# hassony2/handobjectconsist

Hardware: AMD Instinct MI355X
Metric: trainmeshwarp iters/sec (render+warp, B=64, 256x256) (higher is better)
Workload: dtype f32; 1 GPU; trainmeshwarp.py consist step, per-GPU B=64, 256x256, hand 778v/1552f + object 1002v/2000f (7104 faces after fill-back), ResNet-18 fp32 (MIOpen convolutions, channels-last, + fused HIP BatchNorm/ReLU/residual/max-pool kernels), Adam; global_batch=64, image_size=256, parallelism=dp1

## Files before the change

### handobjectconsist_amd/_lib.py

```python
import ctypes
import os

import torch

_HERE = os.path.dirname(os.path.abspath(__file__))
LIB_PATH = os.environ.get("HOC_LIB_PATH") or os.path.join(_HERE, "libmeshraster_hip.so")
ABI_VERSION = 9
FLAG_REFERENCE_ALGO = 1
FLAG_SPARSE_TILES = 2
FLAG_OUTPUT_ZEROED = 4
FLAG_TILE_PER_WORKGROUP = 8
FLAG_TILE_LIST_CLEARED = 16
FLAG_FORCE_PARTS = 1 << 24
FLAG_ONE_WORKGROUP_PER_IMAGE = 32 << 24
FLAG_PARTS_IN_ONE_LAUNCH = 64 << 24
FLAG_PLAIN_DIVISIONS = 4096 << 8
FLAG_FORCE_GATHER = 32 << 8
FLAG_COUNT_PIXEL_MAP_TERMS = 1024 << 8
CRITERION_L1 = 0
CRITERION_L2 = 1
DTYPE_F32, DTYPE_BF16, DTYPE_U8 = 0, 1, 2
DTYPE_CODES = {torch.float32: DTYPE_F32, torch.bfloat16: DTYPE_BF16, torch.uint8: DTYPE_U8}
IMAGE_DTYPES = (torch.float32, torch.bfloat16)
MASK_DTYPES = (torch.float32, torch.uint8)
# ... 71 lines not shown
    "mr_flow_pair_forward_tiles_typed": (_I, [_P] * 4 + [_L] + [_P] * 12 + [_I, _P, _L, _P, _P, _P, _I, _I, _I, _I, _F, _F, _F, _P, _P, _L, _L, _P, _I, _I, _I]),
    "mr_flow_pair_forward_grad_tiles_typed": (_I, [_P] * 4 + [_L] + [_P] * 12 + [_I, _P, _L, _P, _P, _P, _I, _I, _I, _I, _F, _F, _F, _P, _P, _L, _L, _P, _P, _P, _P, _P, _I, _I, _I]),
    "mr_pair_step_struct_bytes": (_L, []),
    "mr_pair_step_field_offsets": (_I, [_P, _I]),
    "mr_pair_step_sizes": (_I, [_P, _P, _P, _P]),
    "mr_pair_step_forward": (_I, [_P, _P]),
    "mr_pair_step_backward": (_I, [_P, _P]),
    "mr_frames_to_batch_workspace_bytes": (_L, [_I, _I, _I]),
    "mr_frames_to_batch": (_I, [_P] * 3 + [_F] * 6 + [_P, _L, _P, _P] + [_I] * 6 + [_P]),
    "mr_frames_to_batch_typed": (_I, [_P] * 3 + [_F] * 6 + [_P, _L, _P, _P] + [_I] * 6 + [_P, _I, _I]),
    "mr_frames_color_augment_workspace_bytes": (_L, [_I, _I, _I]),
    "mr_frames_color_augment": (_I, [_P] * 7 + [_L, _I, _I, _I, _P]),
    "mr_jpeg_info": (_I, [_P, _L, _P]),
    "mr_jpeg_packed_bytes": (_L, [_I] * 5),
    "mr_jpeg_entropy_decode": (_I, [_P, _L, _P, _L]),
    "mr_jpeg_reconstruct_workspace_bytes": (_L, [_I] * 6),
    "mr_jpeg_reconstruct": (_I, [_P] + [_I] * 6 + [_P, _P, _L, _P]),
    "mr_png_packed_bytes": (_L, [_I] * 3),
    "mr_png_unfilter_workspace_bytes": (_L, [_I] * 4),
    "mr_png_unfilter": (_I, [_P] + [_I] * 4 + [_P, _P, _P]),
    "mr_bn_act_forward": (_I, [_P] * 6 + [_F, _I, _I, _I, _P, _I, _I, _I, _P]),
    "mr_bn_act_backward_workspace_bytes": (_L, [_I, _I]),
    "mr_bn_act_backward": (_I, [_P] * 8 + [_F, _I, _I, _I] + [_P] * 5 + [_L, _I, _I, _I, _P]),
    "mr_stem_pool_forward": (_I, [_P] * 5 + [_F, _I, _I, _P, _P, _I, _I, _I, _I, _P]),
    "mr_stem_pool_backward_workspace_bytes": (_L, [_I, _I, _I, _I]),
    "mr_stem_pool_backward": (_I, [_P] * 8 + [_F, _I, _I] + [_P] * 4 + [_L, _I, _I, _I, _I, _P]),
}

_lib = None


def load():
    global _lib
    if _lib is not None:
        return _lib
    if not os.path.exists(LIB_PATH):
        raise RuntimeError(
            f"{LIB_PATH} is missing: the HIP extension has not been built. Run "
            "`python -c 'import __graft_entry__ as g; g.build()'` (or `python handobjectconsist_amd/build.py`). "
            "There is no CPU / PyTorch fallback for the render + warp path."
        )
    lib = ctypes.CDLL(LIB_PATH)
    for name, (res, args) in SIGNATURES.items():
        try:
            fn = getattr(lib, name)
        except AttributeError as e:
            raise RuntimeError(f"{LIB_PATH} does not export {name}; rebuild it") from e
# ... 86 lines not shown
```

### handobjectconsist_amd/csrc/frozen_bn.hip

```cpp
#include "mr_common.hpp"

namespace mr {

__device__ __forceinline__ float relu_nan(float z) { return z > 0.0f ? z : (z != z ? z : 0.0f); }


struct BnParams {
    const void* x;
    const void* residual;
    const float* weight;
    const float* bias;
    const float* mean;
    const float* var;
    float eps;
    int relu;
    int N, C, HW, split;
    void* y;
    const void* grad_y;
    const void* grad_y2;
    void* grad_x;
    void* grad_residual;
    float* partial;
};

// ... 184 lines not shown
#pragma unroll
        for (int i = 0; i < 4; i++) { red[threadIdx.x][i] = sg[i]; red[threadIdx.x][4 + i] = sgx[i]; }
        __syncthreads();
        if (threadIdx.x < groups) {
            float t[8] = {0, 0, 0, 0, 0, 0, 0, 0};
            for (int r = 0; r < rows; r++)
#pragma unroll
                for (int i = 0; i < 8; i++) t[i] += red[r * groups + threadIdx.x][i];
#pragma unroll
            for (int i = 0; i < 4; i++) {
                p.partial[(int64_t)(c0 + i) * gridDim.x + blockIdx.x] = t[i];
                p.partial[(int64_t)(p.C + c0 + i) * gridDim.x + blockIdx.x] = t[4 + i];
            }
        }
    }
}

static inline bool bn_nhwc_ok(int C) { return C >= 4 && C <= 1024 && (1024 % C) == 0; }

static inline int bn_nhwc_blocks(int64_t pixels, int C) {
    const int rows = 256 / (C / 4);
    const int64_t need = (pixels + rows - 1) / rows;
    return (int)(need < BN_NHWC_BLOCKS ? (need < 1 ? 1 : need) : BN_NHWC_BLOCKS);
}

static inline int bn_split(int N, int C) {
    int s = (4096 + C - 1) / C;
    if (s < 1) s = 1;
    if (s > N) s = N;
    return s;
}

static inline bool bn_aligned(const void* p, int bytes) { return (reinterpret_cast<uintptr_t>(p) & (uintptr_t)(bytes - 1)) == 0; }

template <bool BACKWARD>
static void bn_launch(const BnParams& p, int act_dtype, bool vec, hipStream_t s) {
    const dim3 grid((unsigned)(p.C * p.split));
    if (act_dtype == 0) {
        if (vec) hipLaunchKernelGGL((bn_act_kernel<float, true, BACKWARD>), grid, dim3(256), 0, s, p);
        else hipLaunchKernelGGL((bn_act_kernel<float, false, BACKWARD>), grid, dim3(256), 0, s, p);
    } else {
        if (vec) hipLaunchKernelGGL((bn_act_kernel<bf16_t, true, BACKWARD>), grid, dim3(256), 0, s, p);
        else hipLaunchKernelGGL((bn_act_kernel<bf16_t, false, BACKWARD>), grid, dim3(256), 0, s, p);
    }
}

// ... 67 lines not shown
    if (channels_last) {
        if (!bn_aligned(x, vb) || !bn_aligned(grad_y, vb) || !bn_aligned(grad_y2, vb) || !bn_aligned(grad_x, vb) ||
            !bn_aligned(residual, vb) ||
            !bn_aligned(grad_residual, vb))
            return MR_ERR_BADARG;
        slots = bn_nhwc_blocks((int64_t)batch_size * plane, channels);
        const dim3 grid((unsigned)slots);
        if (act_dtype == 0) hipLaunchKernelGGL((bn_act_nhwc_kernel<float, true>), grid, dim3(256), 0, (hipStream_t)stream, p);
        else hipLaunchKernelGGL((bn_act_nhwc_kernel<bf16_t, true>), grid, dim3(256), 0, (hipStream_t)stream, p);
    } else {
        const bool vec = plane % 4 == 0 && bn_aligned(x, vb) && bn_aligned(grad_y, vb) && bn_aligned(grad_y2, vb) &&
                         bn_aligned(grad_x, vb) &&
                         bn_aligned(residual, vb) && bn_aligned(grad_residual, vb);
        bn_launch<true>(p, act_dtype, vec, (hipStream_t)stream);
    }
    MR_CHECK_LAUNCH();
    if (want_params) {
        hipLaunchKernelGGL(bn_finish_kernel, dim3((unsigned)channels), dim3(256), 0, (hipStream_t)stream, p.partial,
                           running_var, eps, grad_weight, grad_bias, channels, slots);
        MR_CHECK_LAUNCH();
    }
    return MR_OK;
}
```

### handobjectconsist_amd/csrc/stem_pool.hip

```cpp
#include "mr_common.hpp"

namespace mr {

__device__ __forceinline__ float sp_relu_nan(float z) { return z > 0.0f ? z : (z != z ? z : 0.0f); }


struct StemParams {
    const void* x;
    const float* weight;
    const float* bias;
    const float* mean;
    const float* var;
    float eps;
    int N, C, H, W, OH, OW;
    int tiles_x, tiles_y;
    void* y;
    const void* grad_y;
    const void* grad_y2;
    void* grad_x;
    float* partial;
    unsigned char* argmax;
};

constexpr int SP_TX = 32, SP_TY = 16;
// ... 305 lines not shown
            sg[i] += gm;
            sgx[i] += gm * d;
        }
        sp_store4<T>(static_cast<T*>(p.grad_x), ip * p.C + c0, out);
    }
    if (p.partial) {
#pragma unroll
        for (int i = 0; i < 4; i++) { red[threadIdx.x][i] = sg[i]; red[threadIdx.x][4 + i] = sgx[i]; }
        __syncthreads();
        if (threadIdx.x < groups) {
            float t[8] = {0, 0, 0, 0, 0, 0, 0, 0};
            for (int r = 0; r < rows; r++)
#pragma unroll
                for (int i = 0; i < 8; i++) t[i] += red[r * groups + threadIdx.x][i];
#pragma unroll
            for (int i = 0; i < 4; i++) {
                p.partial[(int64_t)(c0 + i) * gridDim.x + blockIdx.x] = t[i];
                p.partial[(int64_t)(p.C + c0 + i) * gridDim.x + blockIdx.x] = t[4 + i];
            }
        }
    }
}

static inline bool sp_nhwc_ok(int C) { return C >= 4 && C <= 1024 && (1024 % C) == 0; }
static inline int sp_nhwc_blocks(int64_t pixels, int C) {
    const int rows = 256 / (C / 4);
    const int64_t need = (pixels + rows - 1) / rows;
    return (int)(need < SP_NHWC_BLOCKS ? (need < 1 ? 1 : need) : SP_NHWC_BLOCKS);
}

static int stem_fill(StemParams& p, const void* x, const float* weight, const float* bias, const float* mean,
                     const float* var, float eps, int N, int C, int H, int W) {
    if (N < 0 || C < 0 || H < 0 || W < 0) return MR_ERR_BADARG;
    p.x = x; p.weight = weight; p.bias = bias; p.mean = mean; p.var = var; p.eps = eps;
    p.N = N; p.C = C; p.H = H; p.W = W;
    p.OH = H > 0 ? (H - 1) / 2 + 1 : 0;
    p.OW = W > 0 ? (W - 1) / 2 + 1 : 0;
    p.tiles_x = (p.OW + SP_TX - 1) / SP_TX;
    p.tiles_y = (p.OH + SP_TY - 1) / SP_TY;
    if ((int64_t)N * C * p.tiles_x * p.tiles_y > 0x7fffffff) return MR_ERR_BADARG;
    return MR_OK;
}

}

extern "C" int mr_stem_pool_forward(const void* x, const float* weight, const float* bias, const float* running_mean,
                                    const float* running_var, float eps, int act_dtype, int channels_last, void* y,
                                    unsigned char* argmax, int batch_size, int channels, int height, int width,
                                    mr_stream_t stream) {
    using namespace mr;
    if (act_dtype != 0 && act_dtype != 1) return MR_ERR_BADARG;
    if (channels_last && channels > 0 && !sp_nhwc_ok(channels)) return MR_ERR_BADARG;
    StemParams p{};
    const int rc = stem_fill(p, x, weight, bias, running_mean, running_var, eps, batch_size, channels, height, width);
    if (rc != MR_OK) return rc;
    if (batch_size == 0 || channels == 0 || height == 0 || width == 0) return MR_OK;
    if (!x || !weight || !bias || !running_mean || !running_var || !y) return MR_ERR_BADARG;
    p.y = y;
    if (channels_last) {
        const uintptr_t am = (uintptr_t)(act_dtype == 0 ? 15 : 7);
        if (!argmax || (reinterpret_cast<uintptr_t>(x) & am) || (reinterpret_cast<uintptr_t>(y) & am) ||
            (reinterpret_cast<uintptr_t>(argmax) & 3))
            return MR_ERR_BADARG;
        p.argmax = argmax;
        const dim3 g((unsigned)sp_nhwc_blocks((int64_t)batch_size * p.OH * p.OW, channels));
        if (act_dtype == 0) hipLaunchKernelGGL(stem_pool_nhwc_forward_kernel<float>, g, dim3(256), 0, (hipStream_t)stream, p);
        else hipLaunchKernelGGL(stem_pool_nhwc_forward_kernel<bf16_t>, g, dim3(256), 0, (hipStream_t)stream, p);
        MR_CHECK_LAUNCH();
        return MR_OK;
    }
    const dim3 grid((unsigned)((int64_t)batch_size * channels * p.tiles_x * p.tiles_y));
    if (act_dtype == 0) hipLaunchKernelGGL(stem_pool_forward_kernel<float>, grid, dim3(256), 0, (hipStream_t)stream, p);
    else hipLaunchKernelGGL(stem_pool_forward_kernel<bf16_t>, grid, dim3(256), 0, (hipStream_t)stream, p);
    MR_CHECK_LAUNCH();
    return MR_OK;
}

extern "C" int64_t mr_stem_pool_backward_workspace_bytes(int batch_size, int channels, int height, int width) {
    using namespace mr;
    StemParams p{};
    if (stem_fill(p, nullptr, nullptr, nullptr, nullptr, nullptr, 0.0f, batch_size, channels, height, width) != MR_OK) return -1;
    const int64_t nchw = (int64_t)batch_size * p.tiles_x * p.tiles_y;
    return (int64_t)2 * channels * (nchw > SP_NHWC_BLOCKS ? nchw : SP_NHWC_BLOCKS) * 4 + 16;
}

extern "C" int mr_stem_pool_backward(const void* grad_y, const void* grad_y2, const void* x, const unsigned char* argmax,
                                     const float* weight, const float* bias, const float* running_mean, const float* running_var, float eps,
                                     int act_dtype, int channels_last, void* grad_x, float* grad_weight,
                                     float* grad_bias, void* workspace, int64_t workspace_bytes, int batch_size,
                                     int channels, int height, int width, mr_stream_t stream) {
    using namespace mr;
    if (act_dtype != 0 && act_dtype != 1) return MR_ERR_BADARG;
    if (channels_last && channels > 0 && !sp_nhwc_ok(channels)) return MR_ERR_BADARG;
    StemParams p{};
    const int rc = stem_fill(p, x, weight, bias, running_mean, running_var, eps, batch_size, channels, height, width);
    if (rc != MR_OK) return rc;
    if (channels == 0) return MR_OK;
    const bool want_params = grad_weight || grad_bias;
    if (batch_size == 0 || height == 0 || width == 0) {
        hipError_t e = hipSuccess;
        if (grad_weight) e = hipMemsetAsync(grad_weight, 0, (size_t)channels * 4, (hipStream_t)stream);
        if (e == hipSuccess && grad_bias) e = hipMemsetAsync(grad_bias, 0, (size_t)channels * 4, (hipStream_t)stream);
        return e == hipSuccess ? MR_OK : (int)e;
    }
    if (!grad_y || !x || !weight || !bias || !running_mean || !running_var || !grad_x) return MR_ERR_BADARG;
    if (want_params &&
        (!workspace || workspace_bytes < mr_stem_pool_backward_workspace_bytes(batch_size, channels, height, width)))
        return MR_ERR_BADARG;
    p.grad_y = grad_y; p.grad_y2 = grad_y2; p.grad_x = grad_x;
    p.partial = want_params ? static_cast<float*>(workspace) : nullptr;
    const int tiles = p.tiles_x * p.tiles_y;
    int64_t slots = (int64_t)batch_size * tiles;
    if (channels_last) {
        const uintptr_t am = (uintptr_t)(act_dtype == 0 ? 15 : 7);
        if (!argmax || (reinterpret_cast<uintptr_t>(x) & am) || (reinterpret_cast<uintptr_t>(grad_y) & am) ||
            (reinterpret_cast<uintptr_t>(grad_y2) & am) ||
            (reinterpret_cast<uintptr_t>(grad_x) & am) || (reinterpret_cast<uintptr_t>(argmax) & 3))
            return MR_ERR_BADARG;
        p.argmax = const_cast<unsigned char*>(argmax);
        slots = sp_nhwc_blocks((int64_t)batch_size * height * width, channels);
        const dim3 g((unsigned)slots);
        if (act_dtype == 0) hipLaunchKernelGGL(stem_pool_nhwc_backward_kernel<float>, g, dim3(256), 0, (hipStream_t)stream, p);
        else hipLaunchKernelGGL(stem_pool_nhwc_backward_kernel<bf16_t>, g, dim3(256), 0, (hipStream_t)stream, p);
    } else {
        const dim3 grid((unsigned)((int64_t)batch_size * channels * tiles));
        if (act_dtype == 0) hipLaunchKernelGGL(stem_pool_backward_kernel<float>, grid, dim3(256), 0, (hipStream_t)stream, p);
        else hipLaunchKernelGGL(stem_pool_backward_kernel<bf16_t>, grid, dim3(256), 0, (hipStream_t)stream, p);
    }
    MR_CHECK_LAUNCH();
    if (want_params) {
        hipLaunchKernelGGL(stem_finish_kernel, dim3((unsigned)channels), dim3(256), 0, (hipStream_t)stream, p.partial,
                           running_var, eps, grad_weight, grad_bias, channels, slots);
        MR_CHECK_LAUNCH();
    }
    return MR_OK;
}
// ... 1 lines not shown
```

### handobjectconsist_amd/models/synthnet.py

```python
import os

import numpy as np
import torch
import torch.nn.functional as F
from torch import nn

from handobjectconsist_amd import _lib
from handobjectconsist_amd.nn import frozen_bn
from handobjectconsist_amd.utils import project as camproject
from handobjectconsist_amd.utils import synth


USE_HIP_BN = os.environ.get("HOC_HIP_BN", "1") == "1"


USE_CHANNELS_LAST = os.environ.get("HOC_CHANNELS_LAST", "1") == "1"


def _fused_bn(bn, x):
    if not (USE_HIP_BN and not bn.training and x.is_cuda):
        return False
    out_dtype = torch.get_autocast_dtype("cuda") if torch.is_autocast_enabled("cuda") else x.dtype
    return out_dtype in (torch.float32, torch.bfloat16)


class BasicBlock(nn.Module):
    expansion = 1

    def __init__(self, inplanes, planes, stride=1, downsample=None):
        super().__init__()
        self.conv1 = nn.Conv2d(inplanes, planes, 3, stride, 1, bias=False)
        self.bn1 = nn.BatchNorm2d(planes)
        self.relu = nn.ReLU(inplace=True)
        self.conv2 = nn.Conv2d(planes, planes, 3, 1, 1, bias=False)
        self.bn2 = nn.BatchNorm2d(planes)
        self.downsample = downsample

    def forward_fused(self, x, x_identity, dup=False):
        residual = x_identity if self.downsample is None else frozen_bn.bn_act(
            self.downsample[0](x_identity), self.downsample[1], relu=False)
        out = frozen_bn.bn_act(self.conv1(x), self.bn1)
        return frozen_bn.bn_act(self.conv2(out), self.bn2, residual=residual, dup=dup)

    def forward(self, x):
        if _fused_bn(self.bn1, x):
            return self.forward_fused(x, x)
        residual = x if self.downsample is None else self.downsample(x)
        out = self.relu(self.bn1(self.conv1(x)))
        out = self.bn2(self.conv2(out))
        return self.relu(out + residual)


class ResNet18Features(nn.Module):

    def __init__(self):
        super().__init__()
        self.inplanes = 64
        self.conv1 = nn.Conv2d(3, 64, kernel_size=7, stride=2, padding=3, bias=False)
        self.bn1 = nn.BatchNorm2d(64)
        self.relu = nn.ReLU(inplace=True)
        self.maxpool = nn.MaxPool2d(kernel_size=3, stride=2, padding=1)
        self.layer1 = self._make_layer(64, 2)
        self.layer2 = self._make_layer(128, 2, stride=2)
        self.layer3 = self._make_layer(256, 2, stride=2)
        self.layer4 = self._make_layer(512, 2, stride=2)
# ... 490 lines not shown
```

### handobjectconsist_amd/nn/frozen_bn.py

```python
import torch

from handobjectconsist_amd import _lib


_ACT_DTYPES = {torch.float32: 0, torch.bfloat16: 1}


def _nhwc_channels_ok(C):
    return 4 <= C <= 1024 and 1024 % C == 0


def _layout(x):
    if (x.dim() == 4 and _nhwc_channels_ok(x.shape[1]) and not x.is_contiguous()
            and x.is_contiguous(memory_format=torch.channels_last)):
        return x, 1
    return x.contiguous(), 0


def _aligned(t, cl):
    if t is not None and cl and t.data_ptr() % (4 * t.element_size()):
        return t.clone(memory_format=torch.preserve_format)
    return t


# ... 38 lines not shown
        fmt = torch.channels_last if cl else torch.contiguous_format
        g = _aligned(grad_y.to(xc.dtype).contiguous(memory_format=fmt), cl)
        g2 = _aligned(grad_y2.to(xc.dtype).contiguous(memory_format=fmt), cl) if grad_y2 is not None else None
        dev = xc.device
        grad_x = torch.empty_like(xc)
        grad_r = torch.empty_like(xc) if (rc is not None and need_r) else None
        grad_w = torch.empty_like(w) if need_w else None
        grad_b = torch.empty_like(b) if need_b else None
        wbytes = int(_lib.load().mr_bn_act_backward_workspace_bytes(N, C))
        work = torch.empty((wbytes,), dtype=torch.uint8, device=dev) if (need_w or need_b) else None
        _lib.call("mr_bn_act_backward", _lib.ptr(g), _lib.ptr(g2), _lib.ptr(xc), _lib.ptr(rc), _lib.ptr(w), _lib.ptr(b), _lib.ptr(m),
                  _lib.ptr(v), eps, int(relu), _ACT_DTYPES[xc.dtype], cl, _lib.ptr(grad_x), _lib.ptr(grad_r), _lib.ptr(grad_w),
                  _lib.ptr(grad_b),
                  _lib.ptr(work), wbytes, N, C, plane, _lib.stream_ptr(dev))
        return (grad_x if need_x else None), grad_r, grad_w, grad_b, None, None, None, None, None


def bn_act(x, bn, residual=None, relu=True, dup=False):
    if bn.training or not bn.track_running_stats:
        raise RuntimeError("bn_act needs frozen BatchNorm statistics (module.eval())")
    return _BnActFunction.apply(x, residual, bn.weight, bn.bias, bn.running_mean, bn.running_var, bn.eps, relu, dup)


class _StemPoolFunction(torch.autograd.Function):
    @staticmethod
    def forward(ctx, x, weight, bias, running_mean, running_var, eps, dup):
        ctx.set_materialize_grads(False)
        _lib.check_cuda(x, weight, bias, running_mean, running_var)
        if x.dim() != 4 or x.dtype not in _ACT_DTYPES:
            raise ValueError("expected an fp32 or bf16 [N, C, H, W] tensor")
        xc, cl = _layout(x)
        xc = _aligned(xc, cl)
        N, C, H, W = xc.shape
        w, b = weight.detach().float().contiguous(), bias.detach().float().contiguous()
        m, v = running_mean.float().contiguous(), running_var.float().contiguous()
        oshape = (N, C, (H - 1) // 2 + 1 if H else 0, (W - 1) // 2 + 1 if W else 0)
        fmt = torch.channels_last if cl else torch.contiguous_format
        y = torch.empty(oshape, dtype=xc.dtype, device=xc.device, memory_format=fmt)
        argmax = torch.empty(oshape, dtype=torch.uint8, device=xc.device, memory_format=fmt) if cl else None
        _lib.call("mr_stem_pool_forward", _lib.ptr(xc), _lib.ptr(w), _lib.ptr(b), _lib.ptr(m), _lib.ptr(v), float(eps),
                  _ACT_DTYPES[xc.dtype], cl, _lib.ptr(y), _lib.ptr(argmax), N, C, H, W, _lib.stream_ptr(xc.device))
        ctx.save_for_backward(xc, w, b, m, v, argmax)
        ctx.cfg = (float(eps), cl)
        return (y, y.view_as(y)) if dup else y

    @staticmethod
    def backward(ctx, grad_y, grad_y2=None):
        xc, w, b, m, v, argmax = ctx.saved_tensors
        eps, cl = ctx.cfg
        N, C, H, W = xc.shape
        need_x, need_w, need_b = ctx.needs_input_grad[:3]
        if grad_y is None:
            grad_y, grad_y2 = grad_y2, None
        if grad_y is None:
            return (None,) * 7
        fmt = torch.channels_last if cl else torch.contiguous_format
        g = _aligned(grad_y.to(xc.dtype).contiguous(memory_format=fmt), cl)
        g2 = _aligned(grad_y2.to(xc.dtype).contiguous(memory_format=fmt), cl) if grad_y2 is not None else None
        grad_x = torch.empty_like(xc)
        grad_w = torch.empty_like(w) if need_w else None
        grad_b = torch.empty_like(b) if need_b else None
        wbytes = int(_lib.load().mr_stem_pool_backward_workspace_bytes(N, C, H, W))
        work = torch.empty((wbytes,), dtype=torch.uint8, device=xc.device) if (need_w or need_b) else None
        _lib.call("mr_stem_pool_backward", _lib.ptr(g), _lib.ptr(g2), _lib.ptr(xc), _lib.ptr(argmax), _lib.ptr(w), _lib.ptr(b),
                  _lib.ptr(m),
                  _lib.ptr(v), eps, _ACT_DTYPES[xc.dtype], cl, _lib.ptr(grad_x), _lib.ptr(grad_w), _lib.ptr(grad_b),
                  _lib.ptr(work), wbytes, N, C, H, W,
                  _lib.stream_ptr(xc.device))
        return (grad_x if need_x else None), grad_w, grad_b, None, None, None, None


def stem_pool(x, bn, dup=False):
    if bn.training or not bn.track_running_stats:
        raise RuntimeError("stem_pool needs frozen BatchNorm statistics (module.eval())")
    return _StemPoolFunction.apply(x, bn.weight, bn.bias, bn.running_mean, bn.running_var, bn.eps, dup)
```

### include/meshraster_hip.h

```cpp
#ifndef MESHRASTER_HIP_H
#define MESHRASTER_HIP_H

#include <stdint.h>

#ifdef __cplusplus
extern "C" {
#endif

#define MR_OK 0
#define MR_ERR_BADARG (-1)
#define MR_ERR_NOTIMPL (-2)

#define MR_FLAG_REFERENCE_ALGO 1
#define MR_FLAG_SPARSE_TILES 2
#define MR_FLAG_OUTPUT_ZEROED 4
#define MR_FLAG_TILE_PER_WORKGROUP 8
#define MR_FLAG_TILE_LIST_CLEARED 16
#define MR_FLAG_FORCE_PARTS (1 << 24)
#define MR_FLAG_ONE_WORKGROUP_PER_IMAGE (32 << 24)
#define MR_FLAG_PARTS_IN_ONE_LAUNCH (64 << 24)
#define MR_FLAG_PLAIN_DIVISIONS (4096 << 8)
#define MR_FLAG_FORCE_GATHER (32 << 8)
#define MR_FLAG_COUNT_PIXEL_MAP_TERMS (1024 << 8)

// ... 466 lines not shown

#define MR_PNG_MAGIC 0x3150524D
#define MR_PNG_HEADER_BYTES 64
#define MR_PNG_BAND_ROWS 64
#define MR_PNG_MAX_SIDE 10752
MR_API int64_t mr_png_packed_bytes(int width, int height, int channels);
MR_API int64_t mr_png_unfilter_workspace_bytes(int num_frames, int width, int height, int channels);
MR_API int mr_png_unfilter(const unsigned char* packed, int num_frames, int width, int height, int channels,
                           unsigned char* frames_out, void* workspace, mr_stream_t stream);

MR_API int mr_bn_act_forward(const void* x, const void* residual, const float* weight, const float* bias,
                             const float* running_mean, const float* running_var, float eps, int relu,
                             int act_dtype, int channels_last, void* y, int batch_size, int channels,
                             int plane, mr_stream_t stream);
MR_API int64_t mr_bn_act_backward_workspace_bytes(int batch_size, int channels);
MR_API int mr_bn_act_backward(const void* grad_y, const void* grad_y2, const void* x, const void* residual,
                              const float* weight, const float* bias, const float* running_mean,
                              const float* running_var, float eps, int relu, int act_dtype,
                              int channels_last, void* grad_x, void* grad_residual, float* grad_weight,
                              float* grad_bias,
                              void* workspace, int64_t workspace_bytes, int batch_size, int channels,
                              int plane, mr_stream_t stream);

MR_API int mr_stem_pool_forward(const void* x, const float* weight, const float* bias,
                                const float* running_mean, const float* running_var, float eps,
                                int act_dtype, int channels_last, void* y, unsigned char* argmax,
                                int batch_size, int channels, int height, int width, mr_stream_t stream);
MR_API int64_t mr_stem_pool_backward_workspace_bytes(int batch_size, int channels, int height, int width);
MR_API int mr_stem_pool_backward(const void* grad_y, const void* grad_y2, const void* x,
                                 const unsigned char* argmax,
                                 const float* weight, const float* bias, const float* running_mean,
                                 const float* running_var, float eps, int act_dtype, int channels_last,
                                 void* grad_x, float* grad_weight, float* grad_bias, void* workspace,
                                 int64_t workspace_bytes, int batch_size, int channels, int height,
                                 int width, mr_stream_t stream);

#ifdef __cplusplus
}
#endif
#endif
```

Baseline: 37.79 iters/s (one optimiser step = 1 data batch + 1 consist batch of B per GPU; roofline.stock_trunk_it_s = the same step with the trunk's BatchNorm/ReLU/max-pool on the stock nn modules).

## Fuse downsample BN into residual BN-add-ReLU and save stem pool records

```diff
diff --git a/handobjectconsist_amd/_lib.py b/handobjectconsist_amd/_lib.py
--- a/handobjectconsist_amd/_lib.py
+++ b/handobjectconsist_amd/_lib.py
@@ -117,7 +117,11 @@
     "mr_bn_act_forward": (_I, [_P] * 6 + [_F, _I, _I, _I, _P, _I, _I, _I, _P]),
     "mr_bn_act_backward_workspace_bytes": (_L, [_I, _I]),
     "mr_bn_act_backward": (_I, [_P] * 8 + [_F, _I, _I, _I] + [_P] * 5 + [_L, _I, _I, _I, _P]),
+    "mr_bn_add_bn_act_forward": (_I, [_P] * 6 + [_F] + [_P] * 4 + [_F, _I, _P, _I, _I, _I, _P]),
+    "mr_bn_add_bn_act_backward_workspace_bytes": (_L, [_I, _I]),
+    "mr_bn_add_bn_act_backward": (_I, [_P] * 8 + [_F] + [_P] * 4 + [_F, _I] + [_P] * 7 + [_L, _I, _I, _I, _P]),
     "mr_stem_pool_forward": (_I, [_P] * 5 + [_F, _I, _I, _P, _P, _I, _I, _I, _I, _P]),
+    "mr_stem_pool_records_bytes": (_L, [_I, _I, _I, _I]),
     "mr_stem_pool_backward_workspace_bytes": (_L, [_I, _I, _I, _I]),
     "mr_stem_pool_backward": (_I, [_P] * 8 + [_F, _I, _I] + [_P] * 4 + [_L, _I, _I, _I, _I, _P]),
 }
diff --git a/handobjectconsist_amd/csrc/frozen_bn.hip b/handobjectconsist_amd/csrc/frozen_bn.hip
--- a/handobjectconsist_amd/csrc/frozen_bn.hip
+++ b/handobjectconsist_amd/csrc/frozen_bn.hip
@@ -230,6 +230,122 @@
     const int rows = 256 / (C / 4);
     const int64_t need = (pixels + rows - 1) / rows;
     return (int)(need < BN_NHWC_BLOCKS ? (need < 1 ? 1 : need) : BN_NHWC_BLOCKS);
+}
+
+struct BnAddParams {
+    const void* x;
+    const void* xd;
+    const float* weight;  const float* bias;  const float* mean;  const float* var;
+    const float* weight_d; const float* bias_d; const float* mean_d; const float* var_d;
+    float eps, eps_d;
+    int N, C, HW;
+    void* y;
+    const void* grad_y;
+    const void* grad_y2;
+    void* grad_x;
+    void* grad_xd;
+    float* partial;
+};
+
+template <typename T, bool BACKWARD>
+__global__ __launch_bounds__(256) void bn_add_bn_act_nhwc_kernel(BnAddParams p) {
+    __shared__ float red[256][13];
+    const int groups = p.C >> 2;
+    const int cg = threadIdx.x % groups, prow = threadIdx.x / groups, rows = 256 / groups;
+    const int c0 = 4 * cg;
+    float mean[4], a[4], b[4], mean_d[4], ad[4], bd[4];
+#pragma unroll
+    for (int i = 0; i < 4; i++) {
+        mean[i] = p.mean[c0 + i];
+        a[i] = p.weight[c0 + i] * (1.0f / sqrtf(p.var[c0 + i] + p.eps));
+        b[i] = p.bias[c0 + i];
+        mean_d[i] = p.mean_d[c0 + i];
+        ad[i] = p.weight_d[c0 + i] * (1.0f / sqrtf(p.var_d[c0 + i] + p.eps_d));
+        bd[i] = p.bias_d[c0 + i];
+    }
+    const int64_t pixels = (int64_t)p.N * p.HW;
+    float sg[4] = {0.0f, 0.0f, 0.0f, 0.0f}, sgx[4] = {0.0f, 0.0f, 0.0f, 0.0f}, sgd[4] = {0.0f, 0.0f, 0.0f, 0.0f};
+    for (int64_t px = (int64_t)blockIdx.x * rows + prow; px < pixels; px += (int64_t)gridDim.x * rows) {
+        const int64_t o = px * p.C + c0;
+        float xv[4], dv[4], gv[4], out[4], outd[4];
+        load4<T>(p.x, o, xv);
+        load4<T>(p.xd, o, dv);
+        if (BACKWARD) {
+            load4<T>(p.grad_y, o, gv);
+            if (p.grad_y2) {
+                float g2[4];
+                load4<T>(p.grad_y2, o, g2);
+#pragma unroll
+                for (int i = 0; i < 4; i++) gv[i] += g2[i];
+            }
+        }
+#pragma unroll
+        for (int i = 0; i < 4; i++) {
+            const float dd = dv[i] - mean_d[i];
+            const float r = dd * ad[i] + bd[i];
+            const float d = xv[i] - mean[i];
+            float z = d * a[i] + b[i];
+            z = z + r;
+            if (!BACKWARD) {
+                out[i] = relu_nan(z);
+            } else {
+                const float g = !(z > 0.0f) ? 0.0f : gv[i];
+                out[i] = g * a[i];
+                outd[i] = g * ad[i];
+                sg[i] += g;
+                sgx[i] += g * d;
+                sgd[i] += g * dd;
+            }
+        }
+        store4<T>(BACKWARD ? p.grad_x : p.y, o, out);
+        if (BACKWARD) store4<T>(p.grad_xd, o, outd);
+    }
+    if (BACKWARD && p.partial) {
+#pragma unroll
+        for (int i = 0; i < 4; i++) { red[threadIdx.x][i] = sg[i]; red[threadIdx.x][4 + i] = sgx[i]; red[threadIdx.x][8 + i] = sgd[i]; }
+        __syncthreads();
+        if (threadIdx.x < groups) {
+            float t[12] = {0, 0, 0, 0, 0, 0, 0, 0, 0, 0, 0, 0};
+            for (int r = 0; r < rows; r++)
+#pragma unroll
+                for (int i = 0; i < 12; i++) t[i] += red[r * groups + threadIdx.x][i];
+#pragma unroll
+            for (int i = 0; i < 4; i++) {
+                p.partial[(int64_t)(c0 + i) * gridDim.x + blockIdx.x] = t[i];
+                p.partial[(int64_t)(p.C + c0 + i) * gridDim.x + blockIdx.x] = t[4 + i];
+                p.partial[(int64_t)(2 * p.C + c0 + i) * gridDim.x + blockIdx.x] = t[8 + i];
+            }
+        }
+    }
+}
+
+__global__ __launch_bounds__(256) void bn_add_finish_kernel(const float* __restrict__ partial, const float* __restrict__ var,
+                                                            float eps, const float* __restrict__ var_d, float eps_d,
+                                                            float* grad_weight, float* grad_bias, float* grad_weight_d,
+                                                            float* grad_bias_d, int C, int slots) {
+    __shared__ float red[3][4];
+    const int c = blockIdx.x;
+    float s0 = 0.0f, s1 = 0.0f, s2 = 0.0f;
+    for (int k = threadIdx.x; k < slots; k += 256) {
+        s0 += partial[(int64_t)c * slots + k];
+        s1 += partial[(int64_t)(C + c) * slots + k];
+        s2 += partial[(int64_t)(2 * C + c) * slots + k];
+    }
+#pragma unroll
+    for (int off = 32; off >= 1; off >>= 1) {
+        s0 += __shfl_down(s0, off);
+        s1 += __shfl_down(s1, off);
+        s2 += __shfl_down(s2, off);
+    }
+    if ((threadIdx.x & 63) == 0) { red[0][threadIdx.x >> 6] = s0; red[1][threadIdx.x >> 6] = s1; red[2][threadIdx.x >> 6] = s2; }
+    __syncthreads();
+    if (threadIdx.x == 0) {
+        const float sum_g = (red[0][0] + red[0][1]) + (red[0][2] + red[0][3]);
+        if (grad_bias) grad_bias[c] = sum_g;
+        if (grad_bias_d) grad_bias_d[c] = sum_g;
+        if (grad_weight) grad_weight[c] = ((red[1][0] + red[1][1]) + (red[1][2] + red[1][3])) * (1.0f / sqrtf(var[c] + eps));
+        if (grad_weight_d) grad_weight_d[c] = ((red[2][0] + red[2][1]) + (red[2][2] + red[2][3])) * (1.0f / sqrtf(var_d[c] + eps_d));
+    }
 }
 
 static inline int bn_split(int N, int C) {
@@ -343,3 +459,84 @@
     }
     return MR_OK;
 }
+
+extern "C" int mr_bn_add_bn_act_forward(const void* x, const void* xd, const float* weight, const float* bias,
+                                        const float* running_mean, const float* running_var, float eps,
+                                        const float* weight_d, const float* bias_d, const float* running_mean_d,
+                                        const float* running_var_d, float eps_d, int act_dtype, void* y, int batch_size,
+                                        int channels, int plane, mr_stream_t stream) {
+    using namespace mr;
+    if (batch_size < 0 || channels < 0 || plane < 0 || (act_dtype != 0 && act_dtype != 1)) return MR_ERR_BADARG;
+    if (channels > 0 && !bn_nhwc_ok(channels)) return MR_ERR_BADARG;
+    if (batch_size == 0 || channels == 0 || plane == 0) return MR_OK;
+    if (!x || !xd || !weight || !bias || !running_mean || !running_var || !weight_d || !bias_d || !running_mean_d ||
+        !running_var_d || !y)
+        return MR_ERR_BADARG;
+    const int vb = act_dtype == 0 ? 16 : 8;
+    if (!bn_aligned(x, vb) || !bn_aligned(xd, vb) || !bn_aligned(y, vb)) return MR_ERR_BADARG;
+    BnAddParams p{};
+    p.x = x; p.xd = xd; p.weight = weight; p.bias = bias; p.mean = running_mean; p.var = running_var; p.eps = eps;
+    p.weight_d = weight_d; p.bias_d = bias_d; p.mean_d = running_mean_d; p.var_d = running_var_d; p.eps_d = eps_d;
+    p.N = batch_size; p.C = channels; p.HW = plane; p.y = y;
+    const dim3 grid((unsigned)bn_nhwc_blocks((int64_t)batch_size * plane, channels));
+    if (act_dtype == 0) hipLaunchKernelGGL((bn_add_bn_act_nhwc_kernel<float, false>), grid, dim3(256), 0, (hipStream_t)stream, p);
+    else hipLaunchKernelGGL((bn_add_bn_act_nhwc_kernel<bf16_t, false>), grid, dim3(256), 0, (hipStream_t)stream, p);
+    MR_CHECK_LAUNCH();
+    return MR_OK;
+}
+
+extern "C" int64_t mr_bn_add_bn_act_backward_workspace_bytes(int batch_size, int channels) {
+    if (batch_size < 0 || channels < 0) return -1;
+    return (int64_t)3 * channels * mr::BN_NHWC_BLOCKS * 4 + 16;
+}
+
+extern "C" int mr_bn_add_bn_act_backward(const void* grad_y, const void* grad_y2, const void* x, const void* xd,
+                                         const float* weight, const float* bias, const float* running_mean,
+                                         const float* running_var, float eps, const float* weight_d, const float* bias_d,
+                                         const float* running_mean_d, const float* running_var_d, float eps_d,
+                                         int act_dtype, void* grad_x, void* grad_xd, float* grad_weight, float* grad_bias,
+                                         float* grad_weight_d, float* grad_bias_d, void* workspace,
+                                         int64_t workspace_bytes, int batch_size, int channels, int plane,
+                                         mr_stream_t stream) {
+    using namespace mr;
+    if (batch_size < 0 || channels < 0 || plane < 0 || (act_dtype != 0 && act_dtype != 1)) return MR_ERR_BADARG;
+    if (channels > 0 && !bn_nhwc_ok(channels)) return MR_ERR_BADARG;
+    if (channels == 0) return MR_OK;
+    if (!weight || !bias || !running_mean || !running_var || !weight_d || !bias_d || !running_mean_d || !running_var_d)
+        return MR_ERR_BADARG;
+    const bool want_params = grad_weight || grad_bias || grad_weight_d || grad_bias_d;
+    if (batch_size == 0 || plane == 0) {
+        float* const outs[4] = {grad_weight, grad_bias, grad_weight_d, grad_bias_d};
+        for (float* o : outs)
+            if (o) {
+                const hipError_t e = hipMemsetAsync(o, 0, (size_t)channels * 4, (hipStream_t)stream);
+                if (e != hipSuccess) return (int)e;
+            }
+        return MR_OK;
+    }
+    if (!grad_y || !x || !xd || !grad_x || !grad_xd) return MR_ERR_BADARG;
+    if (want_params && (!workspace || workspace_bytes < mr_bn_add_bn_act_backward_workspace_bytes(batch_size, channels)))
+        return MR_ERR_BADARG;
+    const int vb = act_dtype == 0 ? 16 : 8;
+    if (!bn_aligned(x, vb) || !bn_aligned(xd, vb) || !bn_aligned(grad_y, vb) || !bn_aligned(grad_y2, vb) ||
+        !bn_aligned(grad_x, vb) || !bn_aligned(grad_xd, vb))
+        return MR_ERR_BADARG;
+    BnAddParams p{};
+    p.x = x; p.xd = xd; p.weight = weight; p.bias = bias; p.mean = running_mean; p.var = running_var; p.eps = eps;
+    p.weight_d = weight_d; p.bias_d = bias_d; p.mean_d = running_mean_d; p.var_d = running_var_d; p.eps_d = eps_d;
+    p.N = batch_size; p.C = channels; p.HW = plane;
+    p.grad_y = grad_y; p.grad_y2 = grad_y2; p.grad_x = grad_x; p.grad_xd = grad_xd;
+    p.partial = want_params ? static_cast<float*>(workspace) : nullptr;
+    const int slots = bn_nhwc_blocks((int64_t)batch_size * plane, channels);
+    const dim3 grid((unsigned)slots);
+    if (act_dtype == 0) hipLaunchKernelGGL((bn_add_bn_act_nhwc_kernel<float, true>), grid, dim3(256), 0, (hipStream_t)stream, p);
+    else hipLaunchKernelGGL((bn_add_bn_act_nhwc_kernel<bf16_t, true>), grid, dim3(256), 0, (hipStream_t)stream, p);
+    MR_CHECK_LAUNCH();
+    if (want_params) {
+        hipLaunchKernelGGL(bn_add_finish_kernel, dim3((unsigned)channels), dim3(256), 0, (hipStream_t)stream, p.partial,
+                           running_var, eps, running_var_d, eps_d, grad_weight, grad_bias, grad_weight_d, grad_bias_d,
+                           channels, slots);
+        MR_CHECK_LAUNCH();
+    }
+    return MR_OK;
+}
diff --git a/handobjectconsist_amd/csrc/stem_pool.hip b/handobjectconsist_amd/csrc/stem_pool.hip
--- a/handobjectconsist_amd/csrc/stem_pool.hip
+++ b/handobjectconsist_amd/csrc/stem_pool.hip
@@ -351,6 +351,167 @@
     }
 }
 
+__device__ __forceinline__ unsigned char* sp_rec_codes(const StemParams& p) {
+    return p.argmax + (int64_t)p.N * p.OH * p.OW * p.C * 4;
+}
+
+template <typename T>
+__global__ __launch_bounds__(256) void stem_pool_rec_forward_kernel(StemParams p) {
+    const int groups = p.C >> 2, cg = threadIdx.x % groups, prow = threadIdx.x / groups, rows = 256 / groups;
+    const int c0 = 4 * cg;
+    float mean[4], a[4], b[4];
+#pragma unroll
+    for (int i = 0; i < 4; i++) stem_consts(p, c0 + i, mean[i], a[i], b[i]);
+    const T* x = static_cast<const T*>(p.x);
+    float* rec_d = reinterpret_cast<float*>(p.argmax);
+    unsigned char* rec_code = sp_rec_codes(p);
+    const int QH = (p.OH + 1) >> 1, QW = (p.OW + 1) >> 1;
+    const int64_t total = (int64_t)p.N * QH * QW;
+    for (int64_t q = (int64_t)blockIdx.x * rows + prow; q < total; q += (int64_t)gridDim.x * rows) {
+        const int qx = (int)(q % QW), qy = (int)((q / QW) % QH), n = (int)(q / ((int64_t)QW * QH));
+        const int oy0 = 2 * qy, ox0 = 2 * qx;
+        float best[2][2][4], bd[2][2][4];
+        unsigned bi[2][2][4];
+#pragma unroll
+        for (int w = 0; w < 4; w++)
+#pragma unroll
+            for (int i = 0; i < 4; i++) { best[w >> 1][w & 1][i] = -__builtin_inff(); bd[w >> 1][w & 1][i] = 0.0f; bi[w >> 1][w & 1][i] = 0; }
+#pragma unroll
+        for (int r = 0; r < 5; r++) {
+            const int iy = 2 * oy0 - 1 + r;
+            if (iy < 0 || iy >= p.H) continue;
+#pragma unroll
+            for (int c = 0; c < 5; c++) {
+                const int ix = 2 * ox0 - 1 + c;
+                if (ix < 0 || ix >= p.W) continue;
+                float xv[4];
+                sp_load4<T>(x, (((int64_t)n * p.H + iy) * p.W + ix) * p.C + c0, xv);
+#pragma unroll
+                for (int i = 0; i < 4; i++) {
+                    const float d = xv[i] - mean[i];
+                    const float v = sp_relu_nan(d * a[i] + b[i]);
+#pragma unroll
+                    for (int wy = 0; wy < 2; wy++) {
+                        const int kh = r - 2 * wy;
+                        if (kh < 0 || kh > 2) continue;
+#pragma unroll
+                        for (int wx = 0; wx < 2; wx++) {
+                            const int kw = c - 2 * wx;
+                            if (kw < 0 || kw > 2) continue;
+                            if (v > best[wy][wx][i] || v != v) { best[wy][wx][i] = v; bd[wy][wx][i] = d; bi[wy][wx][i] = (unsigned)(kh * 3 + kw); }
+                        }
+                    }
+                }
+            }
+        }
+#pragma unroll
+        for (int wy = 0; wy < 2; wy++)
+#pragma unroll
+            for (int wx = 0; wx < 2; wx++) {
+                const int oy = oy0 + wy, ox = ox0 + wx;
+                if (oy >= p.OH || ox >= p.OW) continue;
+                const int64_t o = (((int64_t)n * p.OH + oy) * p.OW + ox) * p.C + c0;
+                sp_store4<T>(static_cast<T*>(p.y), o, best[wy][wx]);
+                *reinterpret_cast<float4*>(rec_d + o) = make_float4(bd[wy][wx][0], bd[wy][wx][1], bd[wy][wx][2], bd[wy][wx][3]);
+                *reinterpret_cast<uchar4*>(rec_code + o) = make_uchar4((unsigned char)bi[wy][wx][0], (unsigned char)bi[wy][wx][1],
+                                                                       (unsigned char)bi[wy][wx][2], (unsigned char)bi[wy][wx][3]);
+            }
+    }
+}
+
+template <typename T>
+__global__ __launch_bounds__(256) void stem_pool_rec_backward_kernel(StemParams p) {
+    __shared__ float red[256][9];
+    const int groups = p.C >> 2, cg = threadIdx.x % groups, prow = threadIdx.x / groups, rows = 256 / groups;
+    const int c0 = 4 * cg;
+    float mean[4], a[4], b[4];
+#pragma unroll
+    for (int i = 0; i < 4; i++) stem_consts(p, c0 + i, mean[i], a[i], b[i]);
+    const T* gy = static_cast<const T*>(p.grad_y);
+    const T* gy2 = static_cast<const T*>(p.grad_y2);
+    const float* rec_d = reinterpret_cast<const float*>(p.argmax);
+    const unsigned char* rec_code = sp_rec_codes(p);
+    const int QH = (p.H >> 1) + 1, QW = (p.W >> 1) + 1;
+    const int64_t total = (int64_t)p.N * QH * QW;
+    float sg[4] = {0.0f, 0.0f, 0.0f, 0.0f}, sgx[4] = {0.0f, 0.0f, 0.0f, 0.0f};
+    for (int64_t q = (int64_t)blockIdx.x * rows + prow; q < total; q += (int64_t)gridDim.x * rows) {
+        const int qx = (int)(q % QW), qy = (int)((q / QW) % QH), n = (int)(q / ((int64_t)QW * QH));
+        float s[2][2][4];
+        unsigned code[2][2][4];
+#pragma unroll
+        for (int j = 0; j < 2; j++)
+#pragma unroll
+            for (int k = 0; k < 2; k++) {
+                const int wy = qy - 1 + j, wx = qx - 1 + k;
+#pragma unroll
+                for (int i = 0; i < 4; i++) { s[j][k][i] = 0.0f; code[j][k][i] = 255u; }
+                if (wy < 0 || wy >= p.OH || wx < 0 || wx >= p.OW) continue;
+                const int64_t o = (((int64_t)n * p.OH + wy) * p.OW + wx) * p.C + c0;
+                const uchar4 id = *reinterpret_cast<const uchar4*>(rec_code + o);
+                const float4 dv = *reinterpret_cast<const float4*>(rec_d + o);
+                const float d[4] = {dv.x, dv.y, dv.z, dv.w};
+                float gv[4];
+                sp_load4<T>(gy, o, gv);
+                if (gy2) {
+                    float g2[4];
+                    sp_load4<T>(gy2, o, g2);
+#pragma unroll
+                    for (int i = 0; i < 4; i++) gv[i] += g2[i];
+                }
+                code[j][k][0] = id.x; code[j][k][1] = id.y; code[j][k][2] = id.z; code[j][k][3] = id.w;
+#pragma unroll
+                for (int i = 0; i < 4; i++) {
+                    const float sv = (d[i] * a[i] + b[i] > 0.0f) ? gv[i] : 0.0f;
+                    s[j][k][i] = sv;
+                    if (j == 1 && k == 1) { sg[i] += sv; sgx[i] += sv * d[i]; }
+                }
+            }
+#pragma unroll
+        for (int pr = 0; pr < 2; pr++) {
+            const int iy = 2 * qy - 1 + pr;
+            if (iy < 0 || iy >= p.H) continue;
+#pragma unroll
+            for (int pc = 0; pc < 2; pc++) {
+                const int ix = 2 * qx - 1 + pc;
+                if (ix < 0 || ix >= p.W) continue;
+                float g[4] = {0.0f, 0.0f, 0.0f, 0.0f}, out[4];
+#pragma unroll
+                for (int dy = 0; dy < 2; dy++) {
+                    const int kh = pr + 2 * dy;
+                    if (kh > 2) continue;
+#pragma unroll
+                    for (int dx = 0; dx < 2; dx++) {
+                        const int kw = pc + 2 * dx;
+                        if (kw > 2) continue;
+                        const unsigned want = (unsigned)(kh * 3 + kw);
+#pragma unroll
+                        for (int i = 0; i < 4; i++) g[i] += code[1 - dy][1 - dx][i] == want ? s[1 - dy][1 - dx][i] : 0.0f;
+                    }
+                }
+#pragma unroll
+                for (int i = 0; i < 4; i++) out[i] = g[i] * a[i];
+                sp_store4<T>(static_cast<T*>(p.grad_x), (((int64_t)n * p.H + iy) * p.W + ix) * p.C + c0, out);
+            }
+        }
+    }
+    if (p.partial) {
+#pragma unroll
+        for (int i = 0; i < 4; i++) { red[threadIdx.x][i] = sg[i]; red[threadIdx.x][4 + i] = sgx[i]; }
+        __syncthreads();
+        if (threadIdx.x < groups) {
+            float t[8] = {0, 0, 0, 0, 0, 0, 0, 0};
+            for (int r = 0; r < rows; r++)
+#pragma unroll
+                for (int i = 0; i < 8; i++) t[i] += red[r * groups + threadIdx.x][i];
+#pragma unroll
+            for (int i = 0; i < 4; i++) {
+                p.partial[(int64_t)(c0 + i) * gridDim.x + blockIdx.x] = t[i];
+                p.partial[(int64_t)(p.C + c0 + i) * gridDim.x + blockIdx.x] = t[4 + i];
+            }
+        }
+    }
+}
+
 static inline bool sp_nhwc_ok(int C) { return C >= 4 && C <= 1024 && (1024 % C) == 0; }
 static inline int sp_nhwc_blocks(int64_t pixels, int C) {
     const int rows = 256 / (C / 4);
@@ -386,6 +547,19 @@
     if (batch_size == 0 || channels == 0 || height == 0 || width == 0) return MR_OK;
     if (!x || !weight || !bias || !running_mean || !running_var || !y) return MR_ERR_BADARG;
     p.y = y;
+    if (channels_last == 2) {
+        const uintptr_t am = (uintptr_t)(act_dtype == 0 ? 15 : 7);
+        if (!argmax || (reinterpret_cast<uintptr_t>(x) & am) || (reinterpret_cast<uintptr_t>(y) & am) ||
+            (reinterpret_cast<uintptr_t>(argmax) & 15))
+            return MR_ERR_BADARG;
+        p.argmax = argmax;
+        const int64_t quads = (int64_t)batch_size * ((p.OH + 1) / 2) * ((p.OW + 1) / 2);
+        const dim3 g((unsigned)sp_nhwc_blocks(quads, channels));
+        if (act_dtype == 0) hipLaunchKernelGGL(stem_pool_rec_forward_kernel<float>, g, dim3(256), 0, (hipStream_t)stream, p);
+        else hipLaunchKernelGGL(stem_pool_rec_forward_kernel<bf16_t>, g, dim3(256), 0, (hipStream_t)stream, p);
+        MR_CHECK_LAUNCH();
+        return MR_OK;
+    }
     if (channels_last) {
         const uintptr_t am = (uintptr_t)(act_dtype == 0 ? 15 : 7);
         if (!argmax || (reinterpret_cast<uintptr_t>(x) & am) || (reinterpret_cast<uintptr_t>(y) & am) ||
@@ -403,6 +577,15 @@
     else hipLaunchKernelGGL(stem_pool_forward_kernel<bf16_t>, grid, dim3(256), 0, (hipStream_t)stream, p);
     MR_CHECK_LAUNCH();
     return MR_OK;
+}
+
+extern "C" int64_t mr_stem_pool_records_bytes(int batch_size, int channels, int height, int width) {
+    using namespace mr;
+    StemParams p{};
+    if (stem_fill(p, nullptr, nullptr, nullptr, nullptr, nullptr, 0.0f, batch_size, channels, height, width) != MR_OK) return -1;
+    if (channels > 0 && !sp_nhwc_ok(channels)) return -1;
+    const int64_t values = (int64_t)batch_size * p.OH * p.OW * channels;
+    return values * 4 + (values + 15) / 16 * 16;
 }
 
 extern "C" int64_t mr_stem_pool_backward_workspace_bytes(int batch_size, int channels, int height, int width) {
@@ -432,7 +615,7 @@
         if (e == hipSuccess && grad_bias) e = hipMemsetAsync(grad_bias, 0, (size_t)channels * 4, (hipStream_t)stream);
         return e == hipSuccess ? MR_OK : (int)e;
     }
-    if (!grad_y || !x || !weight || !bias || !running_mean || !running_var || !grad_x) return MR_ERR_BADARG;
+    if (!grad_y || (!x && channels_last != 2) || !weight || !bias || !running_mean || !running_var || !grad_x) return MR_ERR_BADARG;
     if (want_params &&
         (!workspace || workspace_bytes < mr_stem_pool_backward_workspace_bytes(batch_size, channels, height, width)))
         return MR_ERR_BADARG;
@@ -440,7 +623,17 @@
     p.partial = want_params ? static_cast<float*>(workspace) : nullptr;
     const int tiles = p.tiles_x * p.tiles_y;
     int64_t slots = (int64_t)batch_size * tiles;
-    if (channels_last) {
+    if (channels_last == 2) {
+        const uintptr_t am = (uintptr_t)(act_dtype == 0 ? 15 : 7);
+        if (!argmax || (reinterpret_cast<uintptr_t>(grad_y) & am) || (reinterpret_cast<uintptr_t>(grad_y2) & am) ||
+            (reinterpret_cast<uintptr_t>(grad_x) & am) || (reinterpret_cast<uintptr_t>(argmax) & 15))
+            return MR_ERR_BADARG;
+        p.argmax = const_cast<unsigned char*>(argmax);
+        slots = sp_nhwc_blocks((int64_t)batch_size * (height / 2 + 1) * (width / 2 + 1), channels);
+        const dim3 g((unsigned)slots);
+        if (act_dtype == 0) hipLaunchKernelGGL(stem_pool_rec_backward_kernel<float>, g, dim3(256), 0, (hipStream_t)stream, p);
+        else hipLaunchKernelGGL(stem_pool_rec_backward_kernel<bf16_t>, g, dim3(256), 0, (hipStream_t)stream, p);
+    } else if (channels_last) {
         const uintptr_t am = (uintptr_t)(act_dtype == 0 ? 15 : 7);
         if (!argmax || (reinterpret_cast<uintptr_t>(x) & am) || (reinterpret_cast<uintptr_t>(grad_y) & am) ||
             (reinterpret_cast<uintptr_t>(grad_y2) & am) ||
diff --git a/handobjectconsist_amd/models/synthnet.py b/handobjectconsist_amd/models/synthnet.py
--- a/handobjectconsist_amd/models/synthnet.py
+++ b/handobjectconsist_amd/models/synthnet.py
@@ -37,10 +37,12 @@
         self.downsample = downsample
 
     def forward_fused(self, x, x_identity, dup=False):
-        residual = x_identity if self.downsample is None else frozen_bn.bn_act(
-            self.downsample[0](x_identity), self.downsample[1], relu=False)
+        if self.downsample is not None:
+            xd = self.downsample[0](x_identity)
+            out = frozen_bn.bn_act(self.conv1(x), self.bn1)
+            return frozen_bn.bn_add_bn_act(self.conv2(out), self.bn2, xd, self.downsample[1], dup=dup)
         out = frozen_bn.bn_act(self.conv1(x), self.bn1)
-        return frozen_bn.bn_act(self.conv2(out), self.bn2, residual=residual, dup=dup)
+        return frozen_bn.bn_act(self.conv2(out), self.bn2, residual=x_identity, dup=dup)
 
     def forward(self, x):
         if _fused_bn(self.bn1, x):
diff --git a/handobjectconsist_amd/nn/frozen_bn.py b/handobjectconsist_amd/nn/frozen_bn.py
--- a/handobjectconsist_amd/nn/frozen_bn.py
+++ b/handobjectconsist_amd/nn/frozen_bn.py
@@ -84,6 +84,68 @@
     return _BnActFunction.apply(x, residual, bn.weight, bn.bias, bn.running_mean, bn.running_var, bn.eps, relu, dup)
 
 
+class _BnAddBnActFunction(torch.autograd.Function):
+
+    @staticmethod
+    def forward(ctx, x, xd, weight, bias, running_mean, running_var, eps, weight_d, bias_d, running_mean_d,
+                running_var_d, eps_d, dup):
+        ctx.set_materialize_grads(False)
+        _lib.check_cuda(x, xd, weight, bias, running_mean, running_var, weight_d, bias_d, running_mean_d, running_var_d)
+        xc, xdc = _aligned(x, 1), _aligned(xd, 1)
+        N, C = xc.shape[:2]
+        plane = xc[0, 0].numel() if N and C else 0
+        f = lambda t: t.detach().float().contiguous()
+        chan = [f(t) for t in (weight, bias, running_mean, running_var, weight_d, bias_d, running_mean_d, running_var_d)]
+        if not all(t.shape == (C,) for t in chan):
+            raise ValueError("channel arrays must be [C]")
+        y = torch.empty_like(xc)
+        _lib.call("mr_bn_add_bn_act_forward", _lib.ptr(xc), _lib.ptr(xdc), *[_lib.ptr(t) for t in chan[:4]], float(eps),
+                  *[_lib.ptr(t) for t in chan[4:]], float(eps_d), _ACT_DTYPES[xc.dtype], _lib.ptr(y), N, C, plane,
+                  _lib.stream_ptr(xc.device))
+        ctx.save_for_backward(xc, xdc, *chan)
+        ctx.cfg = (float(eps), float(eps_d), N, C, plane)
+        return (y, y.view_as(y)) if dup else y
+
+    @staticmethod
+    def backward(ctx, grad_y, grad_y2=None):
+        xc, xdc, *chan = ctx.saved_tensors
+        eps, eps_d, N, C, plane = ctx.cfg
+        need = ctx.needs_input_grad
+        need_x, need_xd, need_w, need_b, need_wd, need_bd = need[0], need[1], need[2], need[3], need[7], need[8]
+        if grad_y is None:
+            grad_y, grad_y2 = grad_y2, None
+        if grad_y is None:
+            return (None,) * 13
+        fmt = torch.channels_last
+        g = _aligned(grad_y.to(xc.dtype).contiguous(memory_format=fmt), 1)
+        g2 = _aligned(grad_y2.to(xc.dtype).contiguous(memory_format=fmt), 1) if grad_y2 is not None else None
+        dev = xc.device
+        grad_x, grad_xd = torch.empty_like(xc), torch.empty_like(xdc)
+        grads = [torch.empty_like(chan[0]) if n else None for n in (need_w, need_b, need_wd, need_bd)]
+        wbytes = int(_lib.load().mr_bn_add_bn_act_backward_workspace_bytes(N, C))
+        work = torch.empty((wbytes,), dtype=torch.uint8, device=dev) if any(t is not None for t in grads) else None
+        _lib.call("mr_bn_add_bn_act_backward", _lib.ptr(g), _lib.ptr(g2), _lib.ptr(xc), _lib.ptr(xdc),
+                  *[_lib.ptr(t) for t in chan[:4]], eps, *[_lib.ptr(t) for t in chan[4:]], eps_d, _ACT_DTYPES[xc.dtype],
+                  _lib.ptr(grad_x), _lib.ptr(grad_xd), *[_lib.ptr(t) for t in grads], _lib.ptr(work), wbytes, N, C, plane,
+                  _lib.stream_ptr(dev))
+        return ((grad_x if need_x else None), (grad_xd if need_xd else None), grads[0], grads[1], None, None, None,
+                grads[2], grads[3], None, None, None, None)
+
+
+def bn_add_bn_act(x, bn, xd, bn_d, dup=False):
+    for m in (bn, bn_d):
+        if m.training or not m.track_running_stats:
+            raise RuntimeError("bn_add_bn_act needs frozen BatchNorm statistics (module.eval())")
+    if xd.shape != x.shape or xd.dtype != x.dtype:
+        raise ValueError("xd must match x")
+    if x.dim() < 2 or x.dtype not in _ACT_DTYPES:
+        raise ValueError("expected fp32 or bf16 [N, C, ...] tensors")
+    if _layout(x)[1] and _layout(xd)[1]:
+        return _BnAddBnActFunction.apply(x, xd, bn.weight, bn.bias, bn.running_mean, bn.running_var, bn.eps, bn_d.weight,
+                                         bn_d.bias, bn_d.running_mean, bn_d.running_var, bn_d.eps, dup)
+    return bn_act(x, bn, residual=bn_act(xd, bn_d, relu=False), dup=dup)
+
+
 class _StemPoolFunction(torch.autograd.Function):
     @staticmethod
     def forward(ctx, x, weight, bias, running_mean, running_var, eps, dup):
@@ -99,36 +161,40 @@
         oshape = (N, C, (H - 1) // 2 + 1 if H else 0, (W - 1) // 2 + 1 if W else 0)
         fmt = torch.channels_last if cl else torch.contiguous_format
         y = torch.empty(oshape, dtype=xc.dtype, device=xc.device, memory_format=fmt)
-        argmax = torch.empty(oshape, dtype=torch.uint8, device=xc.device, memory_format=fmt) if cl else None
+        layout = 2 if cl else 0
+        records = None
+        if cl:
+            rbytes = int(_lib.load().mr_stem_pool_records_bytes(N, C, H, W))
+            records = torch.empty((rbytes,), dtype=torch.uint8, device=xc.device)
         _lib.call("mr_stem_pool_forward", _lib.ptr(xc), _lib.ptr(w), _lib.ptr(b), _lib.ptr(m), _lib.ptr(v), float(eps),
-                  _ACT_DTYPES[xc.dtype], cl, _lib.ptr(y), _lib.ptr(argmax), N, C, H, W, _lib.stream_ptr(xc.device))
-        ctx.save_for_backward(xc, w, b, m, v, argmax)
-        ctx.cfg = (float(eps), cl)
+                  _ACT_DTYPES[xc.dtype], layout, _lib.ptr(y), _lib.ptr(records), N, C, H, W, _lib.stream_ptr(xc.device))
+        ctx.save_for_backward(None if cl else xc, w, b, m, v, records)
+        ctx.cfg = (float(eps), layout, tuple(xc.shape), xc.dtype, xc.device)
         return (y, y.view_as(y)) if dup else y
 
     @staticmethod
     def backward(ctx, grad_y, grad_y2=None):
-        xc, w, b, m, v, argmax = ctx.saved_tensors
-        eps, cl = ctx.cfg
-        N, C, H, W = xc.shape
+        xc, w, b, m, v, records = ctx.saved_tensors
+        eps, layout, shape, dtype, dev = ctx.cfg
+        N, C, H, W = shape
         need_x, need_w, need_b = ctx.needs_input_grad[:3]
         if grad_y is None:
             grad_y, grad_y2 = grad_y2, None
         if grad_y is None:
             return (None,) * 7
-        fmt = torch.channels_last if cl else torch.contiguous_format
-        g = _aligned(grad_y.to(xc.dtype).contiguous(memory_format=fmt), cl)
-        g2 = _aligned(grad_y2.to(xc.dtype).contiguous(memory_format=fmt), cl) if grad_y2 is not None else None
-        grad_x = torch.empty_like(xc)
+        fmt = torch.channels_last if layout else torch.contiguous_format
+        g = _aligned(grad_y.to(dtype).contiguous(memory_format=fmt), layout)
+        g2 = _aligned(grad_y2.to(dtype).contiguous(memory_format=fmt), layout) if grad_y2 is not None else None
+        grad_x = torch.empty(shape, dtype=dtype, device=dev, memory_format=fmt)
         grad_w = torch.empty_like(w) if need_w else None
         grad_b = torch.empty_like(b) if need_b else None
         wbytes = int(_lib.load().mr_stem_pool_backward_workspace_bytes(N, C, H, W))
-        work = torch.empty((wbytes,), dtype=torch.uint8, device=xc.device) if (need_w or need_b) else None
-        _lib.call("mr_stem_pool_backward", _lib.ptr(g), _lib.ptr(g2), _lib.ptr(xc), _lib.ptr(argmax), _lib.ptr(w), _lib.ptr(b),
+        work = torch.empty((wbytes,), dtype=torch.uint8, device=dev) if (need_w or need_b) else None
+        _lib.call("mr_stem_pool_backward", _lib.ptr(g), _lib.ptr(g2), _lib.ptr(xc), _lib.ptr(records), _lib.ptr(w), _lib.ptr(b),
                   _lib.ptr(m),
-                  _lib.ptr(v), eps, _ACT_DTYPES[xc.dtype], cl, _lib.ptr(grad_x), _lib.ptr(grad_w), _lib.ptr(grad_b),
+                  _lib.ptr(v), eps, _ACT_DTYPES[dtype], layout, _lib.ptr(grad_x), _lib.ptr(grad_w), _lib.ptr(grad_b),
                   _lib.ptr(work), wbytes, N, C, H, W,
-                  _lib.stream_ptr(xc.device))
+                  _lib.stream_ptr(dev))
         return (grad_x if need_x else None), grad_w, grad_b, None, None, None, None
 
 
diff --git a/include/meshraster_hip.h b/include/meshraster_hip.h
--- a/include/meshraster_hip.h
+++ b/include/meshraster_hip.h
@@ -512,10 +512,26 @@
                               void* workspace, int64_t workspace_bytes, int batch_size, int channels,
                               int plane, mr_stream_t stream);
 
+MR_API int mr_bn_add_bn_act_forward(const void* x, const void* xd, const float* weight, const float* bias,
+                                    const float* running_mean, const float* running_var, float eps,
+                                    const float* weight_d, const float* bias_d, const float* running_mean_d,
+                                    const float* running_var_d, float eps_d, int act_dtype, void* y,
+                                    int batch_size, int channels, int plane, mr_stream_t stream);
+MR_API int64_t mr_bn_add_bn_act_backward_workspace_bytes(int batch_size, int channels);
+MR_API int mr_bn_add_bn_act_backward(const void* grad_y, const void* grad_y2, const void* x, const void* xd,
+                                     const float* weight, const float* bias, const float* running_mean,
+                                     const float* running_var, float eps, const float* weight_d,
+                                     const float* bias_d, const float* running_mean_d, const float* running_var_d,
+                                     float eps_d, int act_dtype, void* grad_x, void* grad_xd, float* grad_weight,
+                                     float* grad_bias, float* grad_weight_d, float* grad_bias_d, void* workspace,
+                                     int64_t workspace_bytes, int batch_size, int channels, int plane,
+                                     mr_stream_t stream);
+
 MR_API int mr_stem_pool_forward(const void* x, const float* weight, const float* bias,
                                 const float* running_mean, const float* running_var, float eps,
                                 int act_dtype, int channels_last, void* y, unsigned char* argmax,
                                 int batch_size, int channels, int height, int width, mr_stream_t stream);
+MR_API int64_t mr_stem_pool_records_bytes(int batch_size, int channels, int height, int width);
 MR_API int64_t mr_stem_pool_backward_workspace_bytes(int batch_size, int channels, int height, int width);
 MR_API int mr_stem_pool_backward(const void* grad_y, const void* grad_y2, const void* x,
                                  const unsigned char* argmax,
```

Measured after the change: 38.38 iters/s (one optimiser step = 1 data batch + 1 consist batch of B per GPU; roofline.stock_trunk_it_s = the same step with the trunk's BatchNorm/ReLU/max-pool on the stock nn modules), median of 6. +1.6%, better.
